# farr/mcmc-ocaml

Measured on NVIDIA B200. Metric: chain-steps/sec, higher is better.
Workload: dtype f64

## Files before the change

### mcmc_ocaml_b200/csrc/kdtree_build2.cu

```cuda
#include <algorithm>
#include <cstdlib>
#include <vector>

#include "common.cuh"
#include "kdtree.cuh"
#include "radix_sort.cuh"
#include "scan.cuh"

namespace mg {

constexpr int V2_MAXLEV = 72;
constexpr int V2_MAXL = 64;
constexpr int V2_EXTRA = 3;
constexpr int V2_TB = 256, V2_ITEMS = 8, V2_TILE = V2_TB * V2_ITEMS;

struct V2Level { int32_t lb, le; };
struct V2Info {
  V2Level lvl[V2_MAXLEV + 1];
  int32_t maxsize[V2_MAXLEV + 1];
  int32_t nnodes;
  int32_t nlevels;
  int32_t sel_active;
  int32_t overflow;
};
struct V2Sel { uint64_t prefix; int32_t shift; int32_t dim; };

struct V2Top {
  int64_t N; int D, min_split; int32_t LC, cap;
  V2Info *info;
  int32_t *nb, *ne, *ndim, *nleft, *nspos; double *nsplit;
  uint64_t *lo, *hi;
  V2Sel *sel; int32_t *kth, *below; uint32_t *hist;
  uint64_t *v, *maxL, *minR; uint8_t *fix; int32_t *nR, *ebegin;
};

__device__ __forceinline__ double ordered_to_f64(uint64_t k) {
  const uint64_t b = (k >> 63) ? (k & 0x7FFFFFFFFFFFFFFFull) : ~k;
  return __longlong_as_double((long long)b);
}

__device__ __forceinline__ uint64_t warp_min_u64(uint64_t v);
__device__ __forceinline__ uint64_t warp_max_u64(uint64_t v);

constexpr int V2_MK = 128;
__global__ void __launch_bounds__(256)
v2_make_keys_kernel(const double *__restrict__ pts, int64_t N, int D, uint64_t *__restrict__ K, int32_t *__restrict__ perm,
                    int32_t *__restrict__ seg, uint64_t *__restrict__ root_lo, uint64_t *__restrict__ root_hi, int *__restrict__ nan_flag) {
  extern __shared__ double v2_mk_tile[];
  __shared__ unsigned long long s_lo[64], s_hi[64];
  const int DP = D | 1;
  if (threadIdx.x < 64) { s_lo[threadIdx.x] = ~0ull; s_hi[threadIdx.x] = 0ull; }
  bool bad = false;
  for (int64_t i0 = (int64_t)blockIdx.x * V2_MK; i0 < N; i0 += (int64_t)gridDim.x * V2_MK) {
    const int cnt = (int)((N - i0 < V2_MK) ? N - i0 : V2_MK);
    const double *src = pts + i0 * D;
// ... 440 lines not shown
    v2_load8(Kin + (int64_t)d0 * t.N, base, t.N, vec, key);
    if (two) v2_load8(Kin + (int64_t)(d0 + 1) * t.N, base, t.N, vec, key2);
#pragma unroll
    for (int k = 0; k < V2_ITEMS; ++k) if (ci[k] >= 0) { sk0[ci[k]] = key[k]; if (two) sk1[ci[k]] = key2[k]; }
    __syncthreads();
#pragma unroll
    for (int h = 0; h < 2; ++h) {
      if (h == 1 && !two) break;
      const int d = d0 + h;
      const uint64_t *sk = h == 0 ? sk0 : sk1;
      uint64_t *co = Kout + (int64_t)d * t.N;
#pragma unroll
      for (int q = 0; q < V2_ITEMS; ++q)
        if (odst[q] >= 0) __stcs(co + odst[q], sk[q * V2_TB + threadIdx.x]);
      uint64_t mnA = ~0ull, mxA = 0ull, mnB = ~0ull, mxB = 0ull;
#pragma unroll
      for (int q = 0; q < V2_ITEMS; ++q) {
        const int c = bch[q];
        if (c < 0) continue;
        const uint64_t x = sk[lpos0 + ((q + threadIdx.x) & (V2_ITEMS - 1))];
        if (c == cA) { mnA = x < mnA ? x : mnA; mxA = x > mxA ? x : mxA; }
        else if (c == cB) { mnB = x < mnB ? x : mnB; mxB = x > mxB ? x : mxB; }
        else { atomicMin((unsigned long long *)lo_next + (int64_t)c * t.D + d, (unsigned long long)x);
               atomicMax((unsigned long long *)hi_next + (int64_t)c * t.D + d, (unsigned long long)x); }
      }
      warp_minmax_flush(cA < 0 ? -1 : cA * t.D, mnA, mxA, lo_next + d, hi_next + d);
      if (__any_sync(0xffffffffu, cB >= 0 && cB != cA))
        warp_minmax_flush((cB < 0 || cB == cA) ? -1 : cB * t.D, mnB, mxB, lo_next + d, hi_next + d);
    }
    __syncthreads();
  }
}

__global__ void v2_split_kernel(V2Top t, int L) {
  const V2Level lv = t.info->lvl[L];
  const int k = blockIdx.x * blockDim.x + threadIdx.x;
  if (k >= lv.le - lv.lb) return;
  const int id = lv.lb + k;
  if (t.ndim[id] < 0) return;
  t.nsplit[id] = 0.5 * (ordered_to_f64(t.maxL[k]) + ordered_to_f64(t.minR[k]));
}

struct V2Bottom {
  int64_t N; int D, min_split, L0;
  const V2Info *info;
  const int32_t *nb, *ne;
  const uint64_t *K; const int32_t *perm_in; int32_t *perm_out;
  int32_t *l_dim, *l_child, *l_begin, *l_end; double *l_split;
  int32_t *cnt;
  int32_t *depth;
  int *overflow;
};

template <int NMAX, int BT>
constexpr size_t v2_bottom_smem(int D) {
  return (size_t)D * NMAX * 8  + (size_t)(BT / 32) * 256 * 4  +
         (size_t)NMAX * 2 * 8  + 64;
}

template <int NMAX, int BT>
__global__ void __launch_bounds__(BT)
v2_bottom_kernel(V2Bottom a) {
  extern __shared__ __align__(16) unsigned char v2_smem[];
  uint64_t *skeys = reinterpret_cast<uint64_t *>(v2_smem);
  uint32_t *hist_all = reinterpret_cast<uint32_t *>(skeys + (size_t)a.D * NMAX);
  uint16_t *ids0 = reinterpret_cast<uint16_t *>(hist_all + (BT / 32) * 256), *ids1 = ids0 + NMAX;
  uint16_t *cb0 = ids1 + NMAX, *ce0 = cb0 + NMAX, *cb1 = ce0 + NMAX, *ce1 = cb1 + NMAX;
  uint16_t *spl = ce1 + NMAX, *sps = spl + NMAX;
  __shared__ int s_scan[BT / 32], s_tot;
  const V2Level lv = a.info->lvl[a.L0];
  const int s = blockIdx.x;
  if (s >= lv.le - lv.lb) return;
  const int g = lv.lb + s;
  const int32_t b = a.nb[g], e = a.ne[g];
  const int n = e - b;
  const int tid = threadIdx.x, lane = tid & 31, warp = tid >> 5, nwarps = BT / 32;
  const unsigned full = 0xffffffffu, lt = (1u << lane) - 1u;
  int32_t *cnt = a.cnt + (size_t)s * V2_MAXL;
  if (n > NMAX || n <= 0) { if (tid == 0) { *a.overflow = 1; a.depth[s] = 0; } return; }
  for (int d = 0; d < a.D; ++d) {
    const uint64_t *col = a.K + (int64_t)d * a.N + b;
    for (int j = tid; j < n; j += BT) skeys[(size_t)d * NMAX + j] = col[j];
  }
  for (int j = tid; j < n; j += BT) ids0[j] = (uint16_t)j;
  if (tid == 0) { cb0[0] = 0; ce0[0] = (uint16_t)n; }
  __syncthreads();
  uint16_t *ids = ids0, *idn = ids1, *cb = cb0, *ce = ce0, *nb_ = cb1, *ne_ = ce1;
  uint32_t *h = hist_all + warp * 256;
  uint64_t *cand = reinterpret_cast<uint64_t *>(h);
  int cur_n = 1, lbase = 0, l = 0, level_max = n;
  const int64_t gbase = 2 * (int64_t)b;
  constexpr int kLaneDimMax = 128;
  constexpr int kTinyMax = 8;
  uint64_t *pair_lo = reinterpret_cast<uint64_t *>(hist_all), *pair_hi = pair_lo + (BT / 32) * 64;
  static_assert((BT / 32) * 64 * 16 <= (BT / 32) * 256 * 4, "pair bounds fit the histogram area");
  for (;;) {
    if (tid == 0) cnt[l] = cur_n;
    const bool pair_mode = cur_n <= nwarps && level_max > kLaneDimMax;
    uint64_t pre_lo[2] = {~0ull, ~0ull}, pre_hi[2] = {0ull, 0ull};
    bool have_pre = false;
    if (pair_mode) {
      for (int pair = warp; pair < cur_n * a.D; pair += nwarps) {
        const int node = pair / a.D, d = pair - node * a.D;
        const int nb0 = cb[node], ne0 = ce[node];
        if (ne0 - nb0 <= kLaneDimMax) continue;
        const uint64_t *col = skeys + (size_t)d * NMAX;
        uint64_t mn = ~0ull, mx = 0ull;
        for (int j = nb0 + lane; j < ne0; j += 32) { const uint64_t k = col[ids[j]]; mn = k < mn ? k : mn; mx = k > mx ? k : mx; }
        mn = warp_min_u64(mn); mx = warp_max_u64(mx);
        if (lane == 0) { pair_lo[node * 64 + d] = mn; pair_hi[node * 64 + d] = mx; }
      }
      __syncthreads();
      if (warp < cur_n && ce[warp] - cb[warp] > kLaneDimMax) {
#pragma unroll
        for (int hh = 0; hh < 2; ++hh) {
          const int d = hh * 32 + lane;
          if (d < a.D) { pre_lo[hh] = pair_lo[warp * 64 + d]; pre_hi[hh] = pair_hi[warp * 64 + d]; }
        }
        have_pre = true;
      }
      __syncthreads();
    }
    for (int node = tid; node < cur_n; node += BT) {
      const int nb0 = cb[node], ne0 = ce[node], m = ne0 - nb0;
      if (m > kTinyMax) continue;
      int sd = -1; double split = 0.0; int spos = ne0;
      uint16_t id[kTinyMax];
#pragma unroll
      for (int j = 0; j < kTinyMax; ++j) id[j] = j < m ? ids[nb0 + j] : (uint16_t)0;
      if (m > 1 && m >= a.min_split) {
        double dx_max = neg_inf(); bool all_eq = true;
        for (int d = 0; d < a.D; ++d) {
          const uint64_t *col = skeys + (size_t)d * NMAX;
          uint64_t mn = ~0ull, mx = 0ull;
#pragma unroll
          for (int j = 0; j < kTinyMax; ++j) if (j < m) { const uint64_t k = col[id[j]]; mn = k < mn ? k : mn; mx = k > mx ? k : mx; }
          if (mn != mx) all_eq = false;
          const double dx = ordered_to_f64(mx) - ordered_to_f64(mn);
          if (dx > dx_max) { sd = d; dx_max = dx; }
        }
        if (all_eq) sd = -1;
        if (sd >= 0) {
          const uint64_t *col = skeys + (size_t)sd * NMAX;
          uint64_t key[kTinyMax];
#pragma unroll
          for (int j = 0; j < kTinyMax; ++j) key[j] = j < m ? col[id[j]] : ~0ull;
          uint64_t v = 0ull;
#pragma unroll
          for (int j = 0; j < kTinyMax; ++j) {
            int r = 0;
#pragma unroll
            for (int i = 0; i < kTinyMax; ++i) r += (i < m && (key[i] < key[j] || (key[i] == key[j] && i < j))) ? 1 : 0;
            if (j < m && r == m / 2) v = key[j];
          }
          int below = 0, eq = 0;
#pragma unroll
          for (int j = 0; j < kTinyMax; ++j) if (j < m) { below += key[j] < v; eq += key[j] == v; }
          int cntL = below + eq;
          const bool fix = cntL == m;
          if (fix) cntL = below;
          spos = nb0 + cntL;
          uint64_t ml = 0ull, mr = ~0ull;
          int lc = 0, rc = 0;
#pragma unroll
          for (int j = 0; j < kTinyMax; ++j) {
            if (j >= m) continue;
            const bool left = fix ? (key[j] < v) : (key[j] <= v);
            if (left) { ml = key[j] > ml ? key[j] : ml; idn[nb0 + lc++] = id[j]; }
            else { mr = key[j] < mr ? key[j] : mr; idn[spos + rc++] = id[j]; }
          }
          split = 0.5 * (ordered_to_f64(ml) + ordered_to_f64(mr));
        }
      }
      if (sd < 0) {
#pragma unroll
        for (int j = 0; j < kTinyMax; ++j) if (j < m) idn[nb0 + j] = id[j];
      }
      spl[node] = sd >= 0 ? 1 : 0; sps[node] = (uint16_t)spos;
      const int64_t gk = gbase + lbase + node;
      a.l_dim[gk] = sd; a.l_split[gk] = split; a.l_begin[gk] = nb0; a.l_end[gk] = ne0; a.l_child[gk] = -1;
    }
    for (int node = warp; node < cur_n; node += nwarps) {
      const int nb0 = cb[node], ne0 = ce[node], m = ne0 - nb0;
      if (m <= kTinyMax) continue;
      int sd = -1; double split = 0.0; int spos = ne0;
      if (m > 1 && m >= a.min_split) {
        uint64_t klo[2] = {~0ull, ~0ull}, khi[2] = {0ull, 0ull};
        bool all_eq = true;
        if (have_pre) {
          klo[0] = pre_lo[0]; klo[1] = pre_lo[1]; khi[0] = pre_hi[0]; khi[1] = pre_hi[1];
        } else if (m <= kLaneDimMax) {
#pragma unroll
          for (int hh = 0; hh < 2; ++hh) {
            const int d = hh * 32 + lane;
            if (hh * 32 >= a.D) break;
            const uint64_t *col = skeys + (size_t)(d < a.D ? d : 0) * NMAX;
            uint64_t mn = ~0ull, mx = 0ull;
            for (int j = nb0; j < ne0; ++j) { const uint64_t k = col[ids[j]]; mn = k < mn ? k : mn; mx = k > mx ? k : mx; }
            if (d < a.D) { klo[hh] = mn; khi[hh] = mx; }
          }
        } else {
          for (int d = 0; d < a.D; ++d) {
            const uint64_t *col = skeys + (size_t)d * NMAX;
            uint64_t mn = ~0ull, mx = 0ull;
            for (int j = nb0 + lane; j < ne0; j += 32) { const uint64_t k = col[ids[j]]; mn = k < mn ? k : mn; mx = k > mx ? k : mx; }
            mn = warp_min_u64(mn); mx = warp_max_u64(mx);
            if ((d & 31) == lane) { klo[d >> 5] = mn; khi[d >> 5] = mx; }
          }
        }
        {
          const bool differs = (lane < a.D && klo[0] != khi[0]) || (lane + 32 < a.D && klo[1] != khi[1]);
          all_eq = !__any_sync(full, differs);
        }
        if (!all_eq) {
          double dx_best = neg_inf(); int d_best = -1;
#pragma unroll
          for (int hh = 0; hh < 2; ++hh) {
            const int d = hh * 32 + lane;
            double dx = neg_inf(); bool ok = false;
            if (d < a.D) { dx = ordered_to_f64(khi[hh]) - ordered_to_f64(klo[hh]); ok = dx > neg_inf(); }
            if (!ok) dx = neg_inf();
            double mxv = dx;
#pragma unroll
            for (int off = 16; off > 0; off >>= 1) { const double o = __shfl_xor_sync(full, mxv, off); mxv = o > mxv ? o : mxv; }
            const unsigned who = __ballot_sync(full, ok && dx == mxv);
            if (who && mxv > dx_best) { dx_best = mxv; d_best = hh * 32 + __ffs(who) - 1; }
          }
          sd = d_best;
        }
        if (sd >= 0) {
          const uint64_t *col = skeys + (size_t)sd * NMAX;
          const uint64_t lo = __shfl_sync(full, klo[sd >> 5], sd & 31), hi = __shfl_sync(full, khi[sd >> 5], sd & 31);
          int shift = ((63 - __clzll((long long)(lo ^ hi))) >> 3) << 3;
          uint64_t prefix = shift >= 56 ? 0ull : (lo >> (shift + 8)) << (shift + 8);
          int kth = m / 2, below_tot = 0, cnt_eq = 0, cand_n = m, cshift = 64;
          uint64_t v = 0ull;
          while (cand_n > 32 && cshift != 0) {
            for (int q = lane; q < 256; q += 32) h[q] = 0u;
            __syncwarp();
            for (int j = nb0 + lane; j < ne0; j += 32) {
              const uint64_t k = col[ids[j]];
              if (shift >= 56 || ((k ^ prefix) >> (shift + 8)) == 0ull) atomicAdd(&h[(unsigned)(k >> shift) & 255u], 1u);
            }
            __syncwarp();
            uint32_t c[8]; uint32_t sum = 0;
#pragma unroll
            for (int q = 0; q < 8; ++q) { c[q] = h[lane * 8 + q]; sum += c[q]; }
            uint32_t incl = sum;
#pragma unroll
            for (int off = 1; off < 32; off <<= 1) { const uint32_t x = __shfl_up_sync(full, incl, off); if (lane >= off) incl += x; }
            const uint32_t excl = incl - sum;
            const bool mine = (uint32_t)kth >= excl && (uint32_t)kth < incl;
            const int src = __ffs(__ballot_sync(full, mine)) - 1;
            int bin = 0; uint32_t below = 0, cn = 0;
            if (mine) {
              uint32_t run = excl;
#pragma unroll
              for (int q = 0; q < 8; ++q) { if ((uint32_t)kth >= run && (uint32_t)kth < run + c[q]) { bin = lane * 8 + q; below = run; cn = c[q]; } run += c[q]; }
            }
            bin = __shfl_sync(full, bin, src); below = __shfl_sync(full, below, src); cn = __shfl_sync(full, cn, src);
            prefix |= (uint64_t)bin << shift;
            kth -= (int)below; below_tot += (int)below; cand_n = (int)cn; cshift = shift; shift -= 8;
            __syncwarp();
          }
          if (cand_n > 32) { v = prefix; cnt_eq = cand_n; }
          else {
            int pos = 0;
            for (int j0 = nb0; j0 < ne0; j0 += 32) {
              const int j = j0 + lane;
              const uint64_t k = j < ne0 ? col[ids[j]] : 0ull;
              const bool match = j < ne0 && (cshift >= 64 || ((k ^ prefix) >> cshift) == 0ull);
              const unsigned mk = __ballot_sync(full, match);
              if (match) cand[pos + __popc(mk & lt)] = k;
              pos += __popc(mk);
            }
            __syncwarp();
            const bool have = lane < cand_n;
            const uint64_t mine = have ? cand[lane] : ~0ull;
            int rank = 0;
            for (int q = 0; q < cand_n; ++q) { const uint64_t o = __shfl_sync(full, mine, q); rank += (o < mine || (o == mine && q < lane)) ? 1 : 0; }
            const int src = __ffs(__ballot_sync(full, have && rank == kth)) - 1;
            v = __shfl_sync(full, mine, src < 0 ? 0 : src);
            below_tot += __popc(__ballot_sync(full, have && mine < v));
            cnt_eq = __popc(__ballot_sync(full, have && mine == v));
            __syncwarp();
          }
          int cntL = below_tot + cnt_eq;
          const bool fix = (cntL == m);
          if (fix) cntL = below_tot;
          spos = nb0 + cntL;
          uint64_t ml = 0ull, mr = ~0ull;
          int lc = 0, rc = 0;
          for (int j0 = nb0; j0 < ne0; j0 += 32) {
            const int j = j0 + lane;
            const bool valid = j < ne0;
            const unsigned id = valid ? ids[j] : 0u;
            const uint64_t k = valid ? col[id] : 0ull;
            const bool left = valid && (fix ? (k < v) : (k <= v)), right = valid && !left;
            if (left) ml = k > ml ? k : ml;
            if (right) mr = k < mr ? k : mr;
            const unsigned Lm = __ballot_sync(full, left), Rm = __ballot_sync(full, right);
            if (left) idn[nb0 + lc + __popc(Lm & lt)] = (uint16_t)id;
            if (right) idn[spos + rc + __popc(Rm & lt)] = (uint16_t)id;
            lc += __popc(Lm); rc += __popc(Rm);
          }
          ml = warp_max_u64(ml); mr = warp_min_u64(mr);
          split = 0.5 * (ordered_to_f64(ml) + ordered_to_f64(mr));
        }
      }
      if (sd < 0) for (int j = nb0 + lane; j < ne0; j += 32) idn[j] = ids[j];
      if (lane == 0) {
        spl[node] = sd >= 0 ? 1 : 0; sps[node] = (uint16_t)spos;
        const int64_t gk = gbase + lbase + node;
        a.l_dim[gk] = sd; a.l_split[gk] = split; a.l_begin[gk] = nb0; a.l_end[gk] = ne0; a.l_child[gk] = -1;
      }
    }
    __syncthreads();
    int carry = 0;
    for (int base = 0; base < cur_n; base += BT) {
      const int node = base + tid;
      const int is = node < cur_n ? spl[node] : 0;
      int incl = is;
#pragma unroll
      for (int off = 1; off < 32; off <<= 1) { const int x = __shfl_up_sync(full, incl, off); if (lane >= off) incl += x; }
      if (lane == 31) s_scan[warp] = incl;
      __syncthreads();
      if (warp == 0) {
        int x = lane < nwarps ? s_scan[lane] : 0, xi = x;
#pragma unroll
        for (int off = 1; off < 32; off <<= 1) { const int y = __shfl_up_sync(full, xi, off); if (lane >= off) xi += y; }
        if (lane < nwarps) s_scan[lane] = xi - x;
        if (lane == nwarps - 1) s_tot = xi;
      }
      __syncthreads();
      const int ex = carry + incl - is + s_scan[warp];
      if (is) {
        const int c = 2 * ex;
        a.l_child[gbase + lbase + node] = c;
        nb_[c] = cb[node]; ne_[c] = sps[node]; nb_[c + 1] = sps[node]; ne_[c + 1] = ce[node];
      }
      carry += s_tot;
      __syncthreads();
    }
    const int nsplit = carry;
    if (nsplit == 0) break;
    lbase += cur_n; cur_n = 2 * nsplit; ++l; level_max = level_max / 2 + 1;
    if (l >= V2_MAXL) { if (tid == 0) *a.overflow = 1; --l; break; }
    { uint16_t *x = ids; ids = idn; idn = x; x = cb; cb = nb_; nb_ = x; x = ce; ce = ne_; ne_ = x; }
    __syncthreads();
  }
  for (int j = tid; j < n; j += BT) a.perm_out[b + j] = a.perm_in[b + idn[j]];
  if (tid == 0) { a.depth[s] = l + 1; for (int q = l + 1; q < V2_MAXL; ++q) cnt[q] = 0; }
}

__global__ void __launch_bounds__(1024)
v2_level_scan_kernel(const int32_t *__restrict__ cnt, int32_t *__restrict__ pre, int nsub, int32_t *__restrict__ totals) {
  const int l = blockIdx.x;
  __shared__ int carry;
  if (threadIdx.x == 0) carry = 0;
  __syncthreads();
  for (int base = 0; base < nsub; base += 1024) {
    const int s = base + threadIdx.x;
    const int v = s < nsub ? cnt[(size_t)s * V2_MAXL + l] : 0;
    int tot;
    const int ex = block_exclusive_scan<1024>(v, &tot);
    const int c = carry;
    if (s < nsub) pre[(size_t)s * V2_MAXL + l] = c + ex;
    __syncthreads();
    if (threadIdx.x == 0) carry = c + tot;
    __syncthreads();
  }
  if (threadIdx.x == 0) totals[l] = carry;
}

struct V2LevelBase { int32_t base[V2_MAXL + 1]; };

__global__ void v2_emit_top_kernel(V2Top t, int64_t nn_top, KdNode *__restrict__ nodes, int32_t *__restrict__ count,
                                   int32_t *__restrict__ begin_out) {
  for (int64_t i = (int64_t)blockIdx.x * blockDim.x + threadIdx.x; i < nn_top; i += (int64_t)gridDim.x * blockDim.x) {
    KdNode nd; nd.split = t.nsplit[i]; nd.left = t.nleft[i]; nd.dim = t.ndim[i];
    nodes[i] = nd; count[i] = t.ne[i] - t.nb[i]; begin_out[i] = t.nb[i];
  }
}

__global__ void __launch_bounds__(256)
v2_emit_bottom_kernel(V2Bottom a, const int32_t *__restrict__ pre, V2LevelBase lb, KdNode *__restrict__ nodes,
                      int32_t *__restrict__ count, int32_t *__restrict__ begin_out) {
  const V2Level lv = a.info->lvl[a.L0];
  const int s = blockIdx.x;
  if (s >= lv.le - lv.lb) return;
  const int g = lv.lb + s;
  const int32_t b = a.nb[g];
  const int32_t *cnt = a.cnt + (size_t)s * V2_MAXL, *pr = pre + (size_t)s * V2_MAXL;
  const int depth = a.depth[s];
  int lstart = 0;
  for (int l = 0; l < depth; ++l) {
    const int c = cnt[l];
    for (int i = threadIdx.x; i < c; i += blockDim.x) {
      const int64_t gk = 2 * (int64_t)b + lstart + i;
      const int gid = l == 0 ? g : lb.base[l] + pr[l] + i;
      const int ch = a.l_child[gk];
      KdNode nd; nd.split = a.l_split[gk]; nd.dim = a.l_dim[gk];
      nd.left = ch < 0 ? -1 : lb.base[l + 1] + pr[l + 1] + ch;
      nodes[gid] = nd; count[gid] = a.l_end[gk] - a.l_begin[gk]; begin_out[gid] = b + a.l_begin[gk];
    }
    lstart += c;
  }
}

static inline int64_t v2_align256(int64_t x) { return (x + 255) & ~255LL; }

template <int NMAX, int BT>
static int v2_launch_bottom(mg_ctx *ctx, const V2Bottom &a, int nsub, int D) {
  const size_t smem = v2_bottom_smem<NMAX, BT>(D);
  MG_CUDA(ctx, cudaFuncSetAttribute(v2_bottom_kernel<NMAX, BT>, cudaFuncAttributeMaxDynamicSharedMemorySize, (int)smem));
  v2_bottom_kernel<NMAX, BT><<<(unsigned)nsub, BT, smem, ctx->stream>>>(a);
  MG_CHECK_LAUNCH(ctx);
  return MG_OK;
}

int build_tree_v2(mg_ctx *ctx, const double *d_pts, int64_t N, int D, const double *low, const double *high, int min_split,
                  mg_kdtree **out) {
  cudaStream_t s = ctx->stream;
  static const size_t smem_cap = [] { const char *e = getenv("MCMC_GPU_KD_SMEM_KB"); return (size_t)(e ? std::max(32, atoi(e)) : 224) * 1024; }();
  const int NMAX = v2_bottom_smem<2048, 1024>(D) <= smem_cap ? 2048 : v2_bottom_smem<1024, 1024>(D) <= smem_cap ? 1024
                   : v2_bottom_smem<512, 512>(D) <= smem_cap ? 512 : 256;
  if (N >= (1LL << 30)) return MG_V2_FALLBACK;
  int L0 = 0;
  { int64_t sz = N; while (sz > NMAX) { sz = sz / 2 + 1; ++L0; } }
  if (L0 + V2_EXTRA >= V2_MAXLEV) return MG_V2_FALLBACK;
  const int32_t LC = (int32_t)std::min<int64_t>(std::max<int64_t>(N, 1), 1LL << std::min(L0 + V2_EXTRA, 30));
  const int64_t cap_top = std::min<int64_t>(2 * N + 2, 2LL * LC * 2 + 4);
  time_begin(ctx);
  kt_reset(ctx, (const void *)v2_scatter_kernel);
  DevBuf<uint64_t> KA, KB, lo, hi, lo2, hi2, v, maxL, minR;
  DevBuf<int32_t> permA, permB, segA, segB, nb, ne, ndim, nleft, nspos, kth, below, nR, ebegin;
  DevBuf<double> nsplit;
  DevBuf<V2Sel> sel; DevBuf<uint32_t> hist; DevBuf<uint8_t> fix; DevBuf<V2Info> info;
  DevBuf<unsigned long long> status; DevBuf<unsigned int> ticket; DevBuf<int> nan_flag;
  const int64_t ntiles = (N + V2_TILE - 1) / V2_TILE;
  MG_CUDA(ctx, KA.alloc((size_t)D * N, s)); MG_CUDA(ctx, KB.alloc((size_t)D * N, s));
  MG_CUDA(ctx, permA.alloc(N, s)); MG_CUDA(ctx, permB.alloc(N, s)); MG_CUDA(ctx, segA.alloc(N, s)); MG_CUDA(ctx, segB.alloc(N, s));
  MG_CUDA(ctx, nb.alloc(cap_top, s)); MG_CUDA(ctx, ne.alloc(cap_top, s)); MG_CUDA(ctx, ndim.alloc(cap_top, s));
  MG_CUDA(ctx, nleft.alloc(cap_top, s)); MG_CUDA(ctx, nspos.alloc(cap_top, s)); MG_CUDA(ctx, nsplit.alloc(cap_top, s));
  MG_CUDA(ctx, lo.alloc((size_t)LC * D, s)); MG_CUDA(ctx, hi.alloc((size_t)LC * D, s));
  MG_CUDA(ctx, lo2.alloc((size_t)LC * D, s)); MG_CUDA(ctx, hi2.alloc((size_t)LC * D, s));
  MG_CUDA(ctx, sel.alloc(LC, s)); MG_CUDA(ctx, kth.alloc(LC, s)); MG_CUDA(ctx, below.alloc(LC, s)); MG_CUDA(ctx, hist.alloc((size_t)LC * 256, s));
  MG_CUDA(ctx, v.alloc(LC, s)); MG_CUDA(ctx, maxL.alloc(LC, s)); MG_CUDA(ctx, minR.alloc(LC, s)); MG_CUDA(ctx, fix.alloc(LC, s));
  MG_CUDA(ctx, nR.alloc(LC, s)); MG_CUDA(ctx, ebegin.alloc(LC, s)); MG_CUDA(ctx, info.alloc(1, s));
  MG_CUDA(ctx, status.alloc((size_t)ntiles, s)); MG_CUDA(ctx, ticket.alloc(1, s)); MG_CUDA(ctx, nan_flag.alloc(1, s));
  MG_CUDA(ctx, cudaMemsetAsync(hist.get(), 0, sizeof(uint32_t) * (size_t)LC * 256, s));
  V2Top t{N, D, min_split, LC, (int32_t)cap_top, info.get(), nb.get(), ne.get(), ndim.get(), nleft.get(), nspos.get(), nsplit.get(),
          lo.get(), hi.get(), sel.get(), kth.get(), below.get(), hist.get(), v.get(), maxL.get(), minR.get(), fix.get(), nR.get(), ebegin.get()};
  const unsigned gtile = (unsigned)ntiles;
  {
    const size_t mk_smem = (size_t)V2_MK * (D | 1) * sizeof(double);
    if (mk_smem > 48 * 1024) MG_CUDA(ctx, cudaFuncSetAttribute(v2_make_keys_kernel, cudaFuncAttributeMaxDynamicSharedMemorySize, (int)mk_smem));
    const int64_t gb = std::min<int64_t>((N + V2_MK - 1) / V2_MK, (int64_t)ctx->sm_count * 16);
    v2_init_kernel<<<1, 32, 0, s>>>(t);
    MG_CHECK_LAUNCH(ctx);
    v2_level_init_kernel<<<1, 64, 0, s>>>(t, 0, t.lo, t.hi);
    MG_CHECK_LAUNCH(ctx);
    MG_CUDA(ctx, cudaMemsetAsync(nan_flag.get(), 0, sizeof(int), s));
    v2_make_keys_kernel<<<(unsigned)gb, 256, mk_smem, s>>>(d_pts, N, D, KA.get(), permA.get(), segA.get(), t.lo, t.hi, nan_flag.get());
    MG_CHECK_LAUNCH(ctx);
  }
  uint64_t *lo_next = lo2.get(), *hi_next = hi2.get();
  uint64_t *Kin = KA.get(), *Kout = KB.get();
  int32_t *pin = permA.get(), *pout = permB.get(), *sin = segA.get(), *sout = segB.get();
  auto run_level = [&](int L) -> int {
    const int64_t nodes_cap = std::min<int64_t>(LC, 1LL << std::min(L, 30));
    const unsigned gnode = (unsigned)((nodes_cap + 127) / 128);
    v2_node_kernel<<<gnode, 128, 0, s>>>(t, L);
    MG_CHECK_LAUNCH(ctx);
    for (int pass = 0; pass < 8; ++pass) {
      v2_hist_kernel<<<gtile, V2_TB, 0, s>>>(t, L, Kin, sin);
      MG_CHECK_LAUNCH(ctx);
      v2_pick_kernel<<<(unsigned)((nodes_cap * 32 + 255) / 256), 256, 0, s>>>(t, L);
      MG_CHECK_LAUNCH(ctx);
// ... 135 lines not shown
```

Measured before the change: 43.26 billion.

## Restructure kd-tree bottom build to block-wide per-position processing with shared radix select

Rewrites the per-subtree bottom kernel so each thread owns fixed positions across levels instead of assigning nodes to warps or threads. Bounds come from grouped lane reductions with shared atomics, medians from a block-shared slot-based radix select plus rank counting for small nodes, and partitioning from one block scan. Keys are staged with async copies into padded shared columns. This aims to cut warp imbalance and serial tiny-node work, but adds many block barriers and atomics per level and changes the shared-memory layout, which can alter the NMAX choice.

```diff
diff --git a/mcmc_ocaml_b200/csrc/kdtree_build2.cu b/mcmc_ocaml_b200/csrc/kdtree_build2.cu
--- a/mcmc_ocaml_b200/csrc/kdtree_build2.cu
+++ b/mcmc_ocaml_b200/csrc/kdtree_build2.cu
@@ -1,6 +1,9 @@
 #include <algorithm>
+#include <climits>
 #include <cstdlib>
 #include <vector>
+
+#include <cuda_pipeline.h>
 
 #include "common.cuh"
 #include "kdtree.cuh"
@@ -547,305 +550,387 @@
   int *overflow;
 };
 
-template <int NMAX, int BT>
+constexpr int V2B_T = 64;
+constexpr int V2B_ITER = 8;
+
+__device__ __forceinline__ unsigned *v2_hi32(uint64_t *p) { return reinterpret_cast<unsigned *>(p) + 1; }
+__device__ __forceinline__ unsigned *v2_lo32(uint64_t *p) { return reinterpret_cast<unsigned *>(p); }
+
+template <int NMAX>
 constexpr size_t v2_bottom_smem(int D) {
-  return (size_t)D * NMAX * 8  + (size_t)(BT / 32) * 256 * 4  +
-         (size_t)NMAX * 2 * 8  + 64;
+  return (size_t)D * (NMAX + 1) * 8  + (size_t)NMAX * 8  +
+         (size_t)NMAX * (3 * 8 + 4)  +
+         (size_t)(NMAX / V2B_T) * 1024  + (size_t)NMAX * 4 * 2 ;
 }
 
 template <int NMAX, int BT>
 __global__ void __launch_bounds__(BT)
 v2_bottom_kernel(V2Bottom a) {
+  constexpr int P = NMAX / BT, NSLOT = NMAX / V2B_T, NW = BT / 32;
+  static_assert(NMAX % BT == 0 && NMAX <= 4096, "positions per thread");
+  constexpr int KS = NMAX + 1;
   extern __shared__ __align__(16) unsigned char v2_smem[];
   uint64_t *skeys = reinterpret_cast<uint64_t *>(v2_smem);
-  uint32_t *hist_all = reinterpret_cast<uint32_t *>(skeys + (size_t)a.D * NMAX);
-  uint16_t *ids0 = reinterpret_cast<uint16_t *>(hist_all + (BT / 32) * 256), *ids1 = ids0 + NMAX;
-  uint16_t *cb0 = ids1 + NMAX, *ce0 = cb0 + NMAX, *cb1 = ce0 + NMAX, *ce1 = cb1 + NMAX;
-  uint16_t *spl = ce1 + NMAX, *sps = spl + NMAX;
-  __shared__ int s_scan[BT / 32], s_tot;
+  uint64_t *kpos = skeys + (size_t)a.D * KS;
+  uint64_t *nA = kpos + NMAX;
+  uint64_t *nB = nA + NMAX;
+  uint64_t *nV = nB + NMAX;
+  uint32_t *hist = reinterpret_cast<uint32_t *>(nV + NMAX);
+  uint64_t *cand = reinterpret_cast<uint64_t *>(hist);
+  int32_t *nS = reinterpret_cast<int32_t *>(hist + NSLOT * 256);
+  uint16_t *ids = reinterpret_cast<uint16_t *>(nS + NMAX), *nbg = ids + NMAX, *nen = nbg + NMAX, *nsp = nen + NMAX;
+  uint16_t *rbase = reinterpret_cast<uint16_t *>(hist), *nchild = rbase + NMAX;
+  static_assert(NSLOT * 1024 >= NMAX * 4, "rbase / nchild fit the histogram area");
+  __shared__ uint64_t s_prefix[NSLOT], s_or[NSLOT], s_and[NSLOT];
+  __shared__ int s_node[NSLOT], s_shift[NSLOT], s_dbit[NSLOT], s_kth[NSLOT], s_below[NSLOT], s_cnt[NSLOT], s_state[NSLOT];
+  __shared__ int s_nslot, s_nactive, s_lmax;
   const V2Level lv = a.info->lvl[a.L0];
   const int s = blockIdx.x;
   if (s >= lv.le - lv.lb) return;
   const int g = lv.lb + s;
   const int32_t b = a.nb[g], e = a.ne[g];
   const int n = e - b;
-  const int tid = threadIdx.x, lane = tid & 31, warp = tid >> 5, nwarps = BT / 32;
-  const unsigned full = 0xffffffffu, lt = (1u << lane) - 1u;
+  const int tid = threadIdx.x, lane = tid & 31, warp = tid >> 5;
+  const unsigned full = 0xffffffffu;
   int32_t *cnt = a.cnt + (size_t)s * V2_MAXL;
   if (n > NMAX || n <= 0) { if (tid == 0) { *a.overflow = 1; a.depth[s] = 0; } return; }
   for (int d = 0; d < a.D; ++d) {
     const uint64_t *col = a.K + (int64_t)d * a.N + b;
-    for (int j = tid; j < n; j += BT) skeys[(size_t)d * NMAX + j] = col[j];
-  }
-  for (int j = tid; j < n; j += BT) ids0[j] = (uint16_t)j;
-  if (tid == 0) { cb0[0] = 0; ce0[0] = (uint16_t)n; }
-  __syncthreads();
-  uint16_t *ids = ids0, *idn = ids1, *cb = cb0, *ce = ce0, *nb_ = cb1, *ne_ = ce1;
-  uint32_t *h = hist_all + warp * 256;
-  uint64_t *cand = reinterpret_cast<uint64_t *>(h);
-  int cur_n = 1, lbase = 0, l = 0, level_max = n;
+    for (int j = tid; j < n; j += BT) __pipeline_memcpy_async(skeys + (size_t)d * KS + j, col + j, sizeof(uint64_t));
+  }
+  __pipeline_commit();
+  int pnode[P], pb[P], pe[P], pcode[P];
+  uint16_t pid[P];
+  uint64_t pkey[P];
+#pragma unroll
+  for (int q = 0; q < P; ++q) {
+    const int j = tid * P + q;
+    if (j < n) ids[j] = (uint16_t)j;
+    pnode[q] = j < n ? 0 : -1; pb[q] = 0; pe[q] = n; pcode[q] = -1; pid[q] = 0; pkey[q] = 0ull;
+  }
+  if (tid == 0) { nbg[0] = 0; nen[0] = (uint16_t)n; nA[0] = 0ull; nB[0] = 0ull; nS[0] = INT_MAX; s_nslot = 0; s_nactive = 0; s_lmax = n; }
+  int cur_n = 1, lbase = 0, l = 0;
   const int64_t gbase = 2 * (int64_t)b;
-  constexpr int kLaneDimMax = 128;
-  constexpr int kTinyMax = 8;
-  uint64_t *pair_lo = reinterpret_cast<uint64_t *>(hist_all), *pair_hi = pair_lo + (BT / 32) * 64;
-  static_assert((BT / 32) * 64 * 16 <= (BT / 32) * 256 * 4, "pair bounds fit the histogram area");
+  __pipeline_wait_prior(0);
+#ifdef MG_KD_BOTTOM_PROF
+  long long prof[8] = {0, 0, 0, 0, 0, 0, 0, 0}, t_last = clock64();
+#define V2B_TICK(i) do { if (tid == 0) { const long long t_ = clock64(); prof[i] += t_ - t_last; t_last = t_; } } while (0)
+  __syncthreads(); V2B_TICK(6);
+#else
+#define V2B_TICK(i) do {} while (0)
+#endif
+  auto finish = [&](int k, uint64_t v, int below, int eq) {
+    const int nb0 = nbg[k], m = nen[k] - nb0;
+    int cntL = below + eq;
+    const bool fix = cntL == m;
+    if (fix) { cntL = below; atomicOr(&nS[k], 256); }
+    nV[k] = v; nsp[k] = (uint16_t)(nb0 + cntL);
+  };
   for (;;) {
+    __syncthreads();
+    V2B_TICK(0);
     if (tid == 0) cnt[l] = cur_n;
-    const bool pair_mode = cur_n <= nwarps && level_max > kLaneDimMax;
-    uint64_t pre_lo[2] = {~0ull, ~0ull}, pre_hi[2] = {0ull, 0ull};
-    bool have_pre = false;
-    if (pair_mode) {
-      for (int pair = warp; pair < cur_n * a.D; pair += nwarps) {
-        const int node = pair / a.D, d = pair - node * a.D;
-        const int nb0 = cb[node], ne0 = ce[node];
-        if (ne0 - nb0 <= kLaneDimMax) continue;
-        const uint64_t *col = skeys + (size_t)d * NMAX;
+    const int level_max = s_lmax;
+    const int pairs = cur_n * a.D;
+    if (pairs <= V2B_ITER * BT) {
+      int G = 1;
+      while (G < 32 && pairs * 2 * G <= BT && 8 * G <= level_max) G *= 2;
+      const int gsh = __ffs(G) - 1, ntask = pairs << gsh;
+      double dxr[V2B_ITER];
+#pragma unroll
+      for (int it = 0; it < V2B_ITER; ++it) {
+        dxr[it] = __longlong_as_double(0x7FF8000000000000ll);
+        if (it * BT >= ntask) break;
+        const int t = it * BT + tid, grp = t >> gsh, gl = t & (G - 1);
         uint64_t mn = ~0ull, mx = 0ull;
-        for (int j = nb0 + lane; j < ne0; j += 32) { const uint64_t k = col[ids[j]]; mn = k < mn ? k : mn; mx = k > mx ? k : mx; }
-        mn = warp_min_u64(mn); mx = warp_max_u64(mx);
-        if (lane == 0) { pair_lo[node * 64 + d] = mn; pair_hi[node * 64 + d] = mx; }
-      }
-      __syncthreads();
-      if (warp < cur_n && ce[warp] - cb[warp] > kLaneDimMax) {
-#pragma unroll
-        for (int hh = 0; hh < 2; ++hh) {
-          const int d = hh * 32 + lane;
-          if (d < a.D) { pre_lo[hh] = pair_lo[warp * 64 + d]; pre_hi[hh] = pair_hi[warp * 64 + d]; }
-        }
-        have_pre = true;
-      }
-      __syncthreads();
-    }
-    for (int node = tid; node < cur_n; node += BT) {
-      const int nb0 = cb[node], ne0 = ce[node], m = ne0 - nb0;
-      if (m > kTinyMax) continue;
-      int sd = -1; double split = 0.0; int spos = ne0;
-      uint16_t id[kTinyMax];
-#pragma unroll
-      for (int j = 0; j < kTinyMax; ++j) id[j] = j < m ? ids[nb0 + j] : (uint16_t)0;
-      if (m > 1 && m >= a.min_split) {
-        double dx_max = neg_inf(); bool all_eq = true;
-        for (int d = 0; d < a.D; ++d) {
-          const uint64_t *col = skeys + (size_t)d * NMAX;
-          uint64_t mn = ~0ull, mx = 0ull;
-#pragma unroll
-          for (int j = 0; j < kTinyMax; ++j) if (j < m) { const uint64_t k = col[id[j]]; mn = k < mn ? k : mn; mx = k > mx ? k : mx; }
-          if (mn != mx) all_eq = false;
-          const double dx = ordered_to_f64(mx) - ordered_to_f64(mn);
-          if (dx > dx_max) { sd = d; dx_max = dx; }
-        }
-        if (all_eq) sd = -1;
-        if (sd >= 0) {
-          const uint64_t *col = skeys + (size_t)sd * NMAX;
-          uint64_t key[kTinyMax];
-#pragma unroll
-          for (int j = 0; j < kTinyMax; ++j) key[j] = j < m ? col[id[j]] : ~0ull;
-          uint64_t v = 0ull;
-#pragma unroll
-          for (int j = 0; j < kTinyMax; ++j) {
-            int r = 0;
-#pragma unroll
-            for (int i = 0; i < kTinyMax; ++i) r += (i < m && (key[i] < key[j] || (key[i] == key[j] && i < j))) ? 1 : 0;
-            if (j < m && r == m / 2) v = key[j];
-          }
-          int below = 0, eq = 0;
-#pragma unroll
-          for (int j = 0; j < kTinyMax; ++j) if (j < m) { below += key[j] < v; eq += key[j] == v; }
-          int cntL = below + eq;
-          const bool fix = cntL == m;
-          if (fix) cntL = below;
-          spos = nb0 + cntL;
-          uint64_t ml = 0ull, mr = ~0ull;
-          int lc = 0, rc = 0;
-#pragma unroll
-          for (int j = 0; j < kTinyMax; ++j) {
-            if (j >= m) continue;
-            const bool left = fix ? (key[j] < v) : (key[j] <= v);
-            if (left) { ml = key[j] > ml ? key[j] : ml; idn[nb0 + lc++] = id[j]; }
-            else { mr = key[j] < mr ? key[j] : mr; idn[spos + rc++] = id[j]; }
-          }
-          split = 0.5 * (ordered_to_f64(ml) + ordered_to_f64(mr));
-        }
-      }
-      if (sd < 0) {
-#pragma unroll
-        for (int j = 0; j < kTinyMax; ++j) if (j < m) idn[nb0 + j] = id[j];
-      }
-      spl[node] = sd >= 0 ? 1 : 0; sps[node] = (uint16_t)spos;
-      const int64_t gk = gbase + lbase + node;
-      a.l_dim[gk] = sd; a.l_split[gk] = split; a.l_begin[gk] = nb0; a.l_end[gk] = ne0; a.l_child[gk] = -1;
-    }
-    for (int node = warp; node < cur_n; node += nwarps) {
-      const int nb0 = cb[node], ne0 = ce[node], m = ne0 - nb0;
-      if (m <= kTinyMax) continue;
-      int sd = -1; double split = 0.0; int spos = ne0;
-      if (m > 1 && m >= a.min_split) {
-        uint64_t klo[2] = {~0ull, ~0ull}, khi[2] = {0ull, 0ull};
-        bool all_eq = true;
-        if (have_pre) {
-          klo[0] = pre_lo[0]; klo[1] = pre_lo[1]; khi[0] = pre_hi[0]; khi[1] = pre_hi[1];
-        } else if (m <= kLaneDimMax) {
-#pragma unroll
-          for (int hh = 0; hh < 2; ++hh) {
-            const int d = hh * 32 + lane;
-            if (hh * 32 >= a.D) break;
-            const uint64_t *col = skeys + (size_t)(d < a.D ? d : 0) * NMAX;
-            uint64_t mn = ~0ull, mx = 0ull;
-            for (int j = nb0; j < ne0; ++j) { const uint64_t k = col[ids[j]]; mn = k < mn ? k : mn; mx = k > mx ? k : mx; }
-            if (d < a.D) { klo[hh] = mn; khi[hh] = mx; }
-          }
-        } else {
-          for (int d = 0; d < a.D; ++d) {
-            const uint64_t *col = skeys + (size_t)d * NMAX;
-            uint64_t mn = ~0ull, mx = 0ull;
-            for (int j = nb0 + lane; j < ne0; j += 32) { const uint64_t k = col[ids[j]]; mn = k < mn ? k : mn; mx = k > mx ? k : mx; }
-            mn = warp_min_u64(mn); mx = warp_max_u64(mx);
-            if ((d & 31) == lane) { klo[d >> 5] = mn; khi[d >> 5] = mx; }
+        bool act = false;
+        int k = 0;
+        if (t < ntask) {
+          k = grp / a.D;
+          const int d = grp - k * a.D, nb0 = nbg[k], ne0 = nen[k], m = ne0 - nb0;
+          act = m > 1 && m >= a.min_split;
+          if (act) {
+            const uint64_t *col = skeys + (size_t)d * KS;
+            for (int j = nb0 + gl; j < ne0; j += G) { const uint64_t x = col[ids[j]]; mn = x < mn ? x : mn; mx = x > mx ? x : mx; }
           }
         }
-        {
-          const bool differs = (lane < a.D && klo[0] != khi[0]) || (lane + 32 < a.D && klo[1] != khi[1]);
-          all_eq = !__any_sync(full, differs);
+        for (int off = G >> 1; off > 0; off >>= 1) {
+          const uint64_t omn = __shfl_xor_sync(full, mn, off), omx = __shfl_xor_sync(full, mx, off);
+          mn = omn < mn ? omn : mn; mx = omx > mx ? omx : mx;
         }
-        if (!all_eq) {
-          double dx_best = neg_inf(); int d_best = -1;
-#pragma unroll
-          for (int hh = 0; hh < 2; ++hh) {
-            const int d = hh * 32 + lane;
-            double dx = neg_inf(); bool ok = false;
-            if (d < a.D) { dx = ordered_to_f64(khi[hh]) - ordered_to_f64(klo[hh]); ok = dx > neg_inf(); }
-            if (!ok) dx = neg_inf();
-            double mxv = dx;
-#pragma unroll
-            for (int off = 16; off > 0; off >>= 1) { const double o = __shfl_xor_sync(full, mxv, off); mxv = o > mxv ? o : mxv; }
-            const unsigned who = __ballot_sync(full, ok && dx == mxv);
-            if (who && mxv > dx_best) { dx_best = mxv; d_best = hh * 32 + __ffs(who) - 1; }
+        if (act && gl == 0) {
+          if (mn != mx) nB[k] = 1ull;
+          const double dx = ordered_to_f64(mx) - ordered_to_f64(mn);
+          if (dx == dx) { atomicMax(v2_hi32(&nA[k]), (unsigned)((uint64_t)__double_as_longlong(dx) >> 32)); dxr[it] = dx; }
+        }
+      }
+      __syncthreads();
+#pragma unroll
+      for (int it = 0; it < V2B_ITER; ++it) {
+        if (it * BT >= ntask) break;
+        if (dxr[it] == dxr[it]) {
+          const int k = ((it * BT + tid) >> gsh) / a.D;
+          const uint64_t x = (uint64_t)__double_as_longlong(dxr[it]);
+          if ((unsigned)(x >> 32) == *v2_hi32(&nA[k])) atomicMax(v2_lo32(&nA[k]), (unsigned)x);
+        }
+      }
+      __syncthreads();
+#pragma unroll
+      for (int it = 0; it < V2B_ITER; ++it) {
+        if (it * BT >= ntask) break;
+        if (dxr[it] == dxr[it]) {
+          const int grp = (it * BT + tid) >> gsh, k = grp / a.D;
+          if ((uint64_t)__double_as_longlong(dxr[it]) == nA[k]) atomicMin(&nS[k], grp - k * a.D);
+        }
+      }
+    } else {
+      for (int k = tid; k < cur_n; k += BT) {
+        const int nb0 = nbg[k], ne0 = nen[k], m = ne0 - nb0;
+        int sd = INT_MAX; uint64_t diff = 0ull;
+        if (m > 1 && m >= a.min_split) {
+          double dx_max = neg_inf();
+          for (int d = 0; d < a.D; ++d) {
+            const uint64_t *col = skeys + (size_t)d * KS;
+            uint64_t mn = ~0ull, mx = 0ull;
+            for (int j = nb0; j < ne0; ++j) { const uint64_t x = col[ids[j]]; mn = x < mn ? x : mn; mx = x > mx ? x : mx; }
+            if (mn != mx) diff = 1ull;
+            const double dx = ordered_to_f64(mx) - ordered_to_f64(mn);
+            if (dx > dx_max) { sd = d; dx_max = dx; }
           }
-          sd = d_best;
         }
-        if (sd >= 0) {
-          const uint64_t *col = skeys + (size_t)sd * NMAX;
-          const uint64_t lo = __shfl_sync(full, klo[sd >> 5], sd & 31), hi = __shfl_sync(full, khi[sd >> 5], sd & 31);
-          int shift = ((63 - __clzll((long long)(lo ^ hi))) >> 3) << 3;
-          uint64_t prefix = shift >= 56 ? 0ull : (lo >> (shift + 8)) << (shift + 8);
-          int kth = m / 2, below_tot = 0, cnt_eq = 0, cand_n = m, cshift = 64;
-          uint64_t v = 0ull;
-          while (cand_n > 32 && cshift != 0) {
-            for (int q = lane; q < 256; q += 32) h[q] = 0u;
-            __syncwarp();
-            for (int j = nb0 + lane; j < ne0; j += 32) {
-              const uint64_t k = col[ids[j]];
-              if (shift >= 56 || ((k ^ prefix) >> (shift + 8)) == 0ull) atomicAdd(&h[(unsigned)(k >> shift) & 255u], 1u);
+        nS[k] = sd; nB[k] = diff;
+      }
+    }
+    __syncthreads();
+    V2B_TICK(1);
+    for (int k = tid; k < cur_n; k += BT) {
+      const int nb0 = nbg[k], ne0 = nen[k], m = ne0 - nb0;
+      const int sd = (m > 1 && m >= a.min_split && nB[k] != 0ull && nS[k] != INT_MAX) ? nS[k] : -1;
+      int code = sd;
+      if (sd >= 0 && m > V2B_T) {
+        const int sl = atomicAdd(&s_nslot, 1);
+        code |= (sl + 1) << 9;
+        s_node[sl] = k; s_kth[sl] = m / 2; s_below[sl] = 0; s_or[sl] = 0ull; s_and[sl] = ~0ull;
+      }
+      nS[k] = code; nA[k] = 0ull; nB[k] = ~0ull;
+      const int64_t gk = gbase + lbase + k;
+      a.l_dim[gk] = sd; a.l_split[gk] = 0.0; a.l_begin[gk] = nb0; a.l_end[gk] = ne0; a.l_child[gk] = -1;
+    }
+    if (tid == 0) s_lmax = 0;
+    __syncthreads();
+    V2B_TICK(2);
+    const int nslot = s_nslot;
+#pragma unroll
+    for (int q = 0; q < P; ++q) {
+      const int j = tid * P + q;
+      int code = -1;
+      if (pnode[q] >= 0) {
+        code = nS[pnode[q]];
+        if (code >= 0) { pid[q] = ids[j]; pkey[q] = skeys[(size_t)(code & 255) * KS + pid[q]]; kpos[j] = pkey[q]; }
+      }
+      pcode[q] = code;
+      if (nslot > 0) {
+        const int sl = code >= 0 ? (code >> 9) - 1 : -1;
+        const int s0 = __shfl_sync(full, sl, 0);
+        if (__all_sync(full, sl == s0)) {
+          if (s0 >= 0) {
+            const unsigned oh = __reduce_or_sync(full, (unsigned)(pkey[q] >> 32)), ol = __reduce_or_sync(full, (unsigned)pkey[q]);
+            const unsigned ah = __reduce_and_sync(full, (unsigned)(pkey[q] >> 32)), al = __reduce_and_sync(full, (unsigned)pkey[q]);
+            if (lane == 0) {
+              atomicOr((unsigned long long *)&s_or[s0], ((unsigned long long)oh << 32) | ol);
+              atomicAnd((unsigned long long *)&s_and[s0], ((unsigned long long)ah << 32) | al);
             }
-            __syncwarp();
-            uint32_t c[8]; uint32_t sum = 0;
-#pragma unroll
-            for (int q = 0; q < 8; ++q) { c[q] = h[lane * 8 + q]; sum += c[q]; }
-            uint32_t incl = sum;
-#pragma unroll
-            for (int off = 1; off < 32; off <<= 1) { const uint32_t x = __shfl_up_sync(full, incl, off); if (lane >= off) incl += x; }
-            const uint32_t excl = incl - sum;
-            const bool mine = (uint32_t)kth >= excl && (uint32_t)kth < incl;
-            const int src = __ffs(__ballot_sync(full, mine)) - 1;
-            int bin = 0; uint32_t below = 0, cn = 0;
-            if (mine) {
-              uint32_t run = excl;
-#pragma unroll
-              for (int q = 0; q < 8; ++q) { if ((uint32_t)kth >= run && (uint32_t)kth < run + c[q]) { bin = lane * 8 + q; below = run; cn = c[q]; } run += c[q]; }
-            }
-            bin = __shfl_sync(full, bin, src); below = __shfl_sync(full, below, src); cn = __shfl_sync(full, cn, src);
-            prefix |= (uint64_t)bin << shift;
-            kth -= (int)below; below_tot += (int)below; cand_n = (int)cn; cshift = shift; shift -= 8;
-            __syncwarp();
           }
-          if (cand_n > 32) { v = prefix; cnt_eq = cand_n; }
-          else {
-            int pos = 0;
-            for (int j0 = nb0; j0 < ne0; j0 += 32) {
-              const int j = j0 + lane;
-              const uint64_t k = j < ne0 ? col[ids[j]] : 0ull;
-              const bool match = j < ne0 && (cshift >= 64 || ((k ^ prefix) >> cshift) == 0ull);
-              const unsigned mk = __ballot_sync(full, match);
-              if (match) cand[pos + __popc(mk & lt)] = k;
-              pos += __popc(mk);
-            }
-            __syncwarp();
-            const bool have = lane < cand_n;
-            const uint64_t mine = have ? cand[lane] : ~0ull;
-            int rank = 0;
-            for (int q = 0; q < cand_n; ++q) { const uint64_t o = __shfl_sync(full, mine, q); rank += (o < mine || (o == mine && q < lane)) ? 1 : 0; }
-            const int src = __ffs(__ballot_sync(full, have && rank == kth)) - 1;
-            v = __shfl_sync(full, mine, src < 0 ? 0 : src);
-            below_tot += __popc(__ballot_sync(full, have && mine < v));
-            cnt_eq = __popc(__ballot_sync(full, have && mine == v));
-            __syncwarp();
+        } else if (sl >= 0) {
+          atomicOr((unsigned long long *)&s_or[sl], (unsigned long long)pkey[q]);
+          atomicAnd((unsigned long long *)&s_and[sl], (unsigned long long)pkey[q]);
+        }
+      }
+    }
+    __syncthreads();
+    V2B_TICK(3);
+    if (nslot > 0) {
+      for (int sl = warp; sl < nslot; sl += NW) {
+        for (int q = lane; q < 256; q += 32) hist[sl * 256 + q] = 0u;
+        if (lane == 0) {
+          const uint64_t dif = s_or[sl] ^ s_and[sl];
+          if (dif == 0ull) {
+            const int k = s_node[sl];
+            finish(k, s_and[sl], 0, nen[k] - nbg[k]);
+            s_state[sl] = 0;
+          } else {
+            const int top = 63 - __clzll((long long)dif);
+            s_dbit[sl] = top + 1;
+            s_shift[sl] = top >= 7 ? top - 7 : 0;
+            s_prefix[sl] = top >= 63 ? 0ull : (s_and[sl] >> (top + 1)) << (top + 1);
+            s_state[sl] = 1;
+            atomicAdd(&s_nactive, 1);
           }
-          int cntL = below_tot + cnt_eq;
-          const bool fix = (cntL == m);
-          if (fix) cntL = below_tot;
-          spos = nb0 + cntL;
-          uint64_t ml = 0ull, mr = ~0ull;
-          int lc = 0, rc = 0;
-          for (int j0 = nb0; j0 < ne0; j0 += 32) {
-            const int j = j0 + lane;
-            const bool valid = j < ne0;
-            const unsigned id = valid ? ids[j] : 0u;
-            const uint64_t k = valid ? col[id] : 0ull;
-            const bool left = valid && (fix ? (k < v) : (k <= v)), right = valid && !left;
-            if (left) ml = k > ml ? k : ml;
-            if (right) mr = k < mr ? k : mr;
-            const unsigned Lm = __ballot_sync(full, left), Rm = __ballot_sync(full, right);
-            if (left) idn[nb0 + lc + __popc(Lm & lt)] = (uint16_t)id;
-            if (right) idn[spos + rc + __popc(Rm & lt)] = (uint16_t)id;
-            lc += __popc(Lm); rc += __popc(Rm);
+        }
+      }
+      __syncthreads();
+      while (s_nactive > 0) {
+#pragma unroll
+        for (int q = 0; q < P; ++q) {
+          const int sl = pcode[q] >= 0 ? (pcode[q] >> 9) - 1 : -1;
+          if (sl < 0 || s_state[sl] != 1) continue;
+          const int dbit = s_dbit[sl];
+          if (dbit < 64 && ((pkey[q] ^ s_prefix[sl]) >> dbit) != 0ull) continue;
+          atomicAdd(&hist[sl * 256 + ((unsigned)(pkey[q] >> s_shift[sl]) & 255u)], 1u);
+        }
+        __syncthreads();
+        for (int sl = warp; sl < nslot; sl += NW) {
+          if (s_state[sl] != 1) continue;
+          uint32_t *h = hist + sl * 256;
+          uint32_t c[8]; uint32_t sum = 0;
+#pragma unroll
+          for (int j = 0; j < 8; ++j) { c[j] = h[lane * 8 + j]; sum += c[j]; h[lane * 8 + j] = 0u; }
+          uint32_t incl = sum;
+#pragma unroll
+          for (int off = 1; off < 32; off <<= 1) { const uint32_t x = __shfl_up_sync(full, incl, off); if (lane >= off) incl += x; }
+          const uint32_t excl = incl - sum, kth = (uint32_t)s_kth[sl];
+          const bool mine = kth >= excl && kth < incl;
+          const int src = __ffs(__ballot_sync(full, mine)) - 1;
+          int bin = 0; uint32_t below = 0, cn = 0;
+          if (mine) {
+            uint32_t run = excl;
+#pragma unroll
+            for (int j = 0; j < 8; ++j) { if (kth >= run && kth < run + c[j]) { bin = lane * 8 + j; below = run; cn = c[j]; } run += c[j]; }
           }
-          ml = warp_max_u64(ml); mr = warp_min_u64(mr);
-          split = 0.5 * (ordered_to_f64(ml) + ordered_to_f64(mr));
+          bin = __shfl_sync(full, bin, src < 0 ? 0 : src); below = __shfl_sync(full, below, src < 0 ? 0 : src);
+          cn = __shfl_sync(full, cn, src < 0 ? 0 : src);
+          if (lane != 0) continue;
+          if (src < 0) { *a.overflow = 1; cn = 0; }
+          const int shift = s_shift[sl];
+          const uint64_t prefix = s_prefix[sl] | ((uint64_t)bin << shift);
+          s_prefix[sl] = prefix; s_kth[sl] = (int)(kth - below); s_below[sl] += (int)below; s_dbit[sl] = shift;
+          if (cn <= (uint32_t)V2B_T || shift == 0) {
+            if (cn > (uint32_t)V2B_T) { finish(s_node[sl], prefix, s_below[sl], (int)cn); s_state[sl] = 0; }
+            else { s_cnt[sl] = 0; s_state[sl] = 2; }
+            atomicSub(&s_nactive, 1);
+          } else {
+            s_shift[sl] = shift >= 8 ? shift - 8 : 0;
+          }
         }
-      }
-      if (sd < 0) for (int j = nb0 + lane; j < ne0; j += 32) idn[j] = ids[j];
-      if (lane == 0) {
-        spl[node] = sd >= 0 ? 1 : 0; sps[node] = (uint16_t)spos;
-        const int64_t gk = gbase + lbase + node;
-        a.l_dim[gk] = sd; a.l_split[gk] = split; a.l_begin[gk] = nb0; a.l_end[gk] = ne0; a.l_child[gk] = -1;
-      }
-    }
-    __syncthreads();
-    int carry = 0;
-    for (int base = 0; base < cur_n; base += BT) {
-      const int node = base + tid;
-      const int is = node < cur_n ? spl[node] : 0;
-      int incl = is;
-#pragma unroll
-      for (int off = 1; off < 32; off <<= 1) { const int x = __shfl_up_sync(full, incl, off); if (lane >= off) incl += x; }
-      if (lane == 31) s_scan[warp] = incl;
+        __syncthreads();
+      }
+#pragma unroll
+      for (int q = 0; q < P; ++q) {
+        const int sl = pcode[q] >= 0 ? (pcode[q] >> 9) - 1 : -1;
+        if (sl < 0 || s_state[sl] != 2) continue;
+        const int dbit = s_dbit[sl];
+        if (dbit < 64 && ((pkey[q] ^ s_prefix[sl]) >> dbit) != 0ull) continue;
+        cand[sl * 128 + atomicAdd(&s_cnt[sl], 1)] = pkey[q];
+      }
       __syncthreads();
-      if (warp == 0) {
-        int x = lane < nwarps ? s_scan[lane] : 0, xi = x;
-#pragma unroll
-        for (int off = 1; off < 32; off <<= 1) { const int y = __shfl_up_sync(full, xi, off); if (lane >= off) xi += y; }
-        if (lane < nwarps) s_scan[lane] = xi - x;
-        if (lane == nwarps - 1) s_tot = xi;
-      }
-      __syncthreads();
-      const int ex = carry + incl - is + s_scan[warp];
-      if (is) {
-        const int c = 2 * ex;
-        a.l_child[gbase + lbase + node] = c;
-        nb_[c] = cb[node]; ne_[c] = sps[node]; nb_[c + 1] = sps[node]; ne_[c + 1] = ce[node];
-      }
-      carry += s_tot;
-      __syncthreads();
-    }
-    const int nsplit = carry;
+    }
+    V2B_TICK(4);
+    auto rank = [&](const uint64_t *list, int m, uint64_t x, int &lt, int &eq) {
+      lt = 0; eq = 0;
+      for (int i = 0; i < m; ++i) { const uint64_t y = list[i]; lt += y < x; eq += y == x; }
+    };
+#pragma unroll
+    for (int q = 0; q < P; ++q) {
+      if (pcode[q] < 0 || (pcode[q] >> 9) != 0) continue;
+      const int m = pe[q] - pb[q], kth = m / 2;
+      int lt, eq;
+      rank(kpos + pb[q], m, pkey[q], lt, eq);
+      if (lt <= kth && kth < lt + eq) finish(pnode[q], pkey[q], lt, eq);
+    }
+    if (nslot > 0) {
+      for (int t = tid; t < nslot * V2B_T; t += BT) {
+        const int sl = t / V2B_T, i = t - sl * V2B_T;
+        if (s_state[sl] != 2 || i >= s_cnt[sl]) continue;
+        const int kth = s_kth[sl];
+        int lt, eq;
+        rank(cand + sl * 128, s_cnt[sl], cand[sl * 128 + i], lt, eq);
+        if (lt <= kth && kth < lt + eq) finish(s_node[sl], cand[sl * 128 + i], s_below[sl] + lt, eq);
+      }
+    }
+    __syncthreads();
+    V2B_TICK(5);
+    int val[P], psp[P], tsum = 0;
+    uint64_t cl[P], cr[P];
+#pragma unroll
+    for (int q = 0; q < P; ++q) {
+      const int j = tid * P + q, k = pnode[q];
+      val[q] = 0; psp[q] = 0; cl[q] = 0ull; cr[q] = ~0ull;
+      bool left = false, right = false;
+      if (k >= 0 && pcode[q] >= 0) {
+        const int code = nS[k];
+        const uint64_t v = nV[k];
+        left = (code & 256) ? pkey[q] < v : pkey[q] <= v;
+        right = !left;
+        psp[q] = nsp[k];
+        val[q] = (right ? 1 : 0) + (j == pb[q] ? 1 << 16 : 0);
+      }
+      tsum += val[q];
+      const int k0 = __shfl_sync(full, k, 0);
+      if (__all_sync(full, k == k0)) {
+        if (k0 >= 0 && pcode[q] >= 0) {
+          const uint64_t ml = warp_max_u64(left ? pkey[q] : 0ull), mr = warp_min_u64(right ? pkey[q] : ~0ull);
+          if (lane == 0) { cl[q] = ml; cr[q] = mr; }
+        }
+      } else if (left) cl[q] = pkey[q];
+      else if (right) cr[q] = pkey[q];
+      if (cl[q] != 0ull) atomicMax(v2_hi32(&nA[k]), (unsigned)(cl[q] >> 32));
+      if (cr[q] != ~0ull) atomicMin(v2_hi32(&nB[k]), (unsigned)(cr[q] >> 32));
+    }
+    int tot;
+    int ex = block_exclusive_scan<BT>(tsum, &tot);
+    int pex[P];
+#pragma unroll
+    for (int q = 0; q < P; ++q) {
+      pex[q] = ex; ex += val[q];
+      const int k = pnode[q];
+      if (cl[q] != 0ull && (unsigned)(cl[q] >> 32) == *v2_hi32(&nA[k])) atomicMax(v2_lo32(&nA[k]), (unsigned)cl[q]);
+      if (cr[q] != ~0ull && (unsigned)(cr[q] >> 32) == *v2_hi32(&nB[k])) atomicMin(v2_lo32(&nB[k]), (unsigned)cr[q]);
+      if (val[q] >> 16) {
+        const int c = 2 * (pex[q] >> 16);
+        rbase[k] = (uint16_t)(pex[q] & 0xffff); nchild[k] = (uint16_t)c;
+        a.l_child[gbase + lbase + k] = c;
+      }
+    }
+    const int nsplit = tot >> 16;
+    __syncthreads();
+#pragma unroll
+    for (int q = 0; q < P; ++q) {
+      const int j = tid * P + q, k = pnode[q];
+      if (k < 0 || pcode[q] < 0) continue;
+      const int sp = psp[q], rb = (pex[q] & 0xffff) - rbase[k];
+      ids[(val[q] & 1) ? sp + rb : j - rb] = pid[q];
+      if (val[q] >> 16) a.l_split[gbase + lbase + k] = 0.5 * (ordered_to_f64(nA[k]) + ordered_to_f64(nB[k]));
+    }
+    __syncthreads();
+#pragma unroll
+    for (int q = 0; q < P; ++q) {
+      const int j = tid * P + q, k = pnode[q];
+      if (k < 0) continue;
+      if (pcode[q] < 0) { pnode[q] = -1; continue; }
+      const int sp = psp[q], c = nchild[k];
+      if (val[q] >> 16) {
+        const int nb0 = pb[q], ne0 = pe[q];
+        nbg[c] = (uint16_t)nb0; nen[c] = (uint16_t)sp; nbg[c + 1] = (uint16_t)sp; nen[c + 1] = (uint16_t)ne0;
+        nA[c] = nA[c + 1] = 0ull; nB[c] = nB[c + 1] = 0ull; nS[c] = nS[c + 1] = INT_MAX;
+        atomicMax(&s_lmax, max(sp - nb0, ne0 - sp));
+      }
+      if (j < sp) { pnode[q] = c; pe[q] = sp; } else { pnode[q] = c + 1; pb[q] = sp; }
+    }
+    if (tid == 0) { s_nslot = 0; s_nactive = 0; }
     if (nsplit == 0) break;
-    lbase += cur_n; cur_n = 2 * nsplit; ++l; level_max = level_max / 2 + 1;
+    lbase += cur_n; cur_n = 2 * nsplit; ++l;
     if (l >= V2_MAXL) { if (tid == 0) *a.overflow = 1; --l; break; }
-    { uint16_t *x = ids; ids = idn; idn = x; x = cb; cb = nb_; nb_ = x; x = ce; ce = ne_; ne_ = x; }
-    __syncthreads();
-  }
-  for (int j = tid; j < n; j += BT) a.perm_out[b + j] = a.perm_in[b + idn[j]];
+  }
+  __syncthreads();
+  V2B_TICK(0);
+  for (int j = tid; j < n; j += BT) a.perm_out[b + j] = a.perm_in[b + ids[j]];
   if (tid == 0) { a.depth[s] = l + 1; for (int q = l + 1; q < V2_MAXL; ++q) cnt[q] = 0; }
+#ifdef MG_KD_BOTTOM_PROF
+  if (tid == 0 && blockIdx.x < 4)
+    printf("v2_bottom prof block %d n %d levels %d: load %lld bounds %lld node %lld stage %lld radix %lld rank %lld split %lld\n",
+           blockIdx.x, n, l + 1, prof[6], prof[1], prof[2], prof[3], prof[4], prof[5], prof[0]);
+#endif
+#undef V2B_TICK
 }
 
 __global__ void __launch_bounds__(1024)
@@ -907,7 +992,7 @@
 
 template <int NMAX, int BT>
 static int v2_launch_bottom(mg_ctx *ctx, const V2Bottom &a, int nsub, int D) {
-  const size_t smem = v2_bottom_smem<NMAX, BT>(D);
+  const size_t smem = v2_bottom_smem<NMAX>(D);
   MG_CUDA(ctx, cudaFuncSetAttribute(v2_bottom_kernel<NMAX, BT>, cudaFuncAttributeMaxDynamicSharedMemorySize, (int)smem));
   v2_bottom_kernel<NMAX, BT><<<(unsigned)nsub, BT, smem, ctx->stream>>>(a);
   MG_CHECK_LAUNCH(ctx);
@@ -918,8 +1003,8 @@
                   mg_kdtree **out) {
   cudaStream_t s = ctx->stream;
   static const size_t smem_cap = [] { const char *e = getenv("MCMC_GPU_KD_SMEM_KB"); return (size_t)(e ? std::max(32, atoi(e)) : 224) * 1024; }();
-  const int NMAX = v2_bottom_smem<2048, 1024>(D) <= smem_cap ? 2048 : v2_bottom_smem<1024, 1024>(D) <= smem_cap ? 1024
-                   : v2_bottom_smem<512, 512>(D) <= smem_cap ? 512 : 256;
+  const int NMAX = v2_bottom_smem<2048>(D) <= smem_cap ? 2048 : v2_bottom_smem<1024>(D) <= smem_cap ? 1024
+                   : v2_bottom_smem<512>(D) <= smem_cap ? 512 : 256;
   if (N >= (1LL << 30)) return MG_V2_FALLBACK;
   int L0 = 0;
   { int64_t sz = N; while (sz > NMAX) { sz = sz / 2 + 1; ++L0; } }
```

Measured after the change: 43.14 billion (median of 6 runs). About the same (-0.3%).
